# lturing/tacotronv2_wavernn_chinese

Measured on AMD Instinct MI355X. Metric: audio ksamples/sec (22.05 kHz, 10-bit RAW WaveRNN, batch=1 per GPU), higher is better.
Workload: dtype f32

## Files before the change

### tacotronv2_wavernn_chinese_amd/csrc/loop_team2.hip

```cpp
#include "device_util.h"
#include "wrnn_internal.h"

#define T2_WGS 32
#define T2_THREADS 512
#define T2_SPIN_MAX 300000u

typedef unsigned long long u64;

namespace {

__device__ __forceinline__ unsigned xcc_id2() {
    unsigned v;
    asm volatile("s_getreg_b32 %0, hwreg(HW_REG_XCC_ID)" : "=s"(v));
    return v & 0xf;
}

__device__ __forceinline__ void st_granule(u64 *base, unsigned idx, unsigned tag, unsigned payload) {
    const u64 v = ((u64)tag << 32) | payload;
    const unsigned off = idx * 8u;
    asm volatile("global_store_dwordx2 %0, %1, %2" ::"v"(off), "v"(v), "s"(base) : "memory");
}
template <int N>
__device__ __forceinline__ void peek_n(const u64 *base, unsigned idx, unsigned stride, u64 (&g)[N]) {
#pragma unroll
    for (int i = 0; i < N; ++i) g[i] = __hip_atomic_load(base + idx + (unsigned)i * stride, __ATOMIC_RELAXED, __HIP_MEMORY_SCOPE_AGENT);
}
template <int N, int SHIFT>
__device__ __forceinline__ bool tags_ok(const u64 (&g)[N], unsigned tag) {
    bool ok = true;
#pragma unroll
    for (int i = 0; i < N; ++i) ok = ok && ((unsigned)(g[i] >> SHIFT) == tag);
    return ok;
}
template <int N, int SHIFT>
__device__ __forceinline__ void finish_n(const u64 *base, unsigned idx, unsigned stride, unsigned tag, u64 (&g)[N], bool &dead,
                                         unsigned *err, unsigned code) {
    unsigned spins = 0;
    while (!dead && !__all(tags_ok<N, SHIFT>(g, tag))) {
        if (++spins > T2_SPIN_MAX) { dead = true; if ((threadIdx.x & 63) == 0) atomicExch(err, code); break; }
        peek_n<N>(base, idx, stride, g);
    }
}

#ifndef T2_STAGGER
#define T2_STAGGER 3
#endif
#ifndef T2_DEFER_OUT
#define T2_DEFER_OUT 0
#endif
#ifndef T2_PRESLEEP
#define T2_PRESLEEP 0
#endif
#ifndef T2_LATE_B
#define T2_LATE_B 2
#endif
__device__ __forceinline__ unsigned take_granule(const u64 *base, unsigned idx, unsigned tag, bool &dead, unsigned *err, unsigned code, u64 (&gb)[1]) {
    u64 ga[1];
#if T2_PRESLEEP
    __builtin_amdgcn_s_sleep(T2_PRESLEEP);
#endif
    peek_n<1>(base, idx, 1, ga);
#if T2_LATE_B == 2
    finish_n<1, 32>(base, idx, 1, tag, ga, dead, err, code);
    return (unsigned)ga[0];
#else
    __builtin_amdgcn_s_sleep(T2_STAGGER);
    peek_n<1>(base, idx, 1, gb);
    if (__all(tags_ok<1, 32>(ga, tag))) {
        unsigned r = (unsigned)ga[0];
#if T2_LATE_B
        asm volatile("" : "+v"(r));
#endif
        return r;
    }
#if T2_LATE_B
    if (__all(tags_ok<1, 32>(gb, tag))) { unsigned r = (unsigned)gb[0]; asm volatile("" : "+v"(r)); return r; }
    u64 gc[1];
    peek_n<1>(base, idx, 1, gc);
    finish_n<1, 32>(base, idx, 1, tag, gc, dead, err, code);
    unsigned r = (unsigned)gc[0];
    asm volatile("" : "+v"(r));
    return r;
#else
    finish_n<1, 32>(base, idx, 1, tag, gb, dead, err, code);
    return (unsigned)gb[0];
#endif
#endif
}
__device__ __forceinline__ void retire_look(u64 (&gb)[1]) {
#if T2_LATE_B
    asm volatile("" ::"v"(gb[0]));
#endif
}

template <int CTRL>
__device__ __forceinline__ float dpp_get(float v) {
    return __int_as_float(__builtin_amdgcn_update_dpp(0, __float_as_int(v), CTRL, 0xf, 0xf, true));
}
__device__ __forceinline__ float row_sum(float v) {
    v += dpp_get<0xB1>(v);
    v += dpp_get<0x4E>(v);
    v += dpp_get<0x141>(v);
    v += dpp_get<0x140>(v);
    return v;
}
__device__ __forceinline__ float wave_max(float v) {
    asm volatile(
        "s_nop 1\n\t"
        "v_max_f32_dpp %0, %0, %0 quad_perm:[1,0,3,2] row_mask:0xf bank_mask:0xf\n\t"
        "s_nop 1\n\t"
        "v_max_f32_dpp %0, %0, %0 quad_perm:[2,3,0,1] row_mask:0xf bank_mask:0xf\n\t"
        "s_nop 1\n\t"
        "v_max_f32_dpp %0, %0, %0 row_half_mirror row_mask:0xf bank_mask:0xf\n\t"
        "s_nop 1\n\t"
        "v_max_f32_dpp %0, %0, %0 row_mirror row_mask:0xf bank_mask:0xf\n\t"
        "s_nop 1\n\t"
        "v_max_f32_dpp %0, %0, %0 row_bcast:15 row_mask:0xa bank_mask:0xf\n\t"
        "s_nop 1\n\t"
        "v_max_f32_dpp %0, %0, %0 row_bcast:31 row_mask:0xc bank_mask:0xf\n\t"
        "s_nop 1"
        : "+v"(v));
    return v;
}

#define XB_PLANE 68
#define XB_VEC (8 * XB_PLANE)
__device__ __forceinline__ int perm(int j) { return ((j >> 2) & 7) * XB_PLANE + (j >> 5) * 4 + (j & 3); }

typedef float f2 __attribute__((ext_vector_type(2)));
__device__ __forceinline__ f2 mk2(float a, float b) { f2 r; r.x = a; r.y = b; return r; }
__device__ __forceinline__ f2 pkfma(f2 a, f2 b, f2 c) { return __builtin_elementwise_fma(a, b, c); }

__device__ __forceinline__ void dot32x3(const float *w, const float *vec, int q, float &o0, float &o1, float &o2) {
    const float4 *p = (const float4 *)vec + q;
    f2 a = mk2(0.f, 0.f), b = mk2(0.f, 0.f), c = mk2(0.f, 0.f);
#pragma unroll
    for (int h = 0; h < 2; ++h) {
        float4 x[4];
#pragma unroll
        for (int k = 0; k < 4; ++k) x[k] = p[(4 * h + k) * (XB_PLANE / 4)];
#pragma unroll
        for (int k = 0; k < 4; ++k) {
            const int kk = 4 * h + k;
            const f2 xl = mk2(x[k].x, x[k].y), xh = mk2(x[k].z, x[k].w);
            a = pkfma(mk2(w[4 * kk + 0], w[4 * kk + 1]), xl, a);
            b = pkfma(mk2(w[32 + 4 * kk + 0], w[32 + 4 * kk + 1]), xl, b);
            c = pkfma(mk2(w[64 + 4 * kk + 0], w[64 + 4 * kk + 1]), xl, c);
            a = pkfma(mk2(w[4 * kk + 2], w[4 * kk + 3]), xh, a);
            b = pkfma(mk2(w[32 + 4 * kk + 2], w[32 + 4 * kk + 3]), xh, b);
            c = pkfma(mk2(w[64 + 4 * kk + 2], w[64 + 4 * kk + 3]), xh, c);
        }
    }
    o0 = a.x + a.y; o1 = b.x + b.y; o2 = c.x + c.y;
}
__device__ __forceinline__ void dot32x3_mixed(const float *w, const float4 *wl_, const float *vec, int q, float &o0, float &o1, float &o2) {
    const float4 *p = (const float4 *)vec + q;
    f2 a = mk2(0.f, 0.f), b = mk2(0.f, 0.f), c = mk2(0.f, 0.f);
#pragma unroll
    for (int h = 0; h < 2; ++h) {
        float4 x[4], wn[4];
#pragma unroll
        for (int k = 0; k < 4; ++k) { x[k] = p[(4 * h + k) * (XB_PLANE / 4)]; wn[k] = wl_[(4 * h + k) * 256]; }
#pragma unroll
        for (int k = 0; k < 4; ++k) {
            const int kk = 4 * h + k;
            const f2 xl = mk2(x[k].x, x[k].y), xh = mk2(x[k].z, x[k].w);
            a = pkfma(mk2(w[4 * kk + 0], w[4 * kk + 1]), xl, a);
            b = pkfma(mk2(w[32 + 4 * kk + 0], w[32 + 4 * kk + 1]), xl, b);
            c = pkfma(mk2(wn[k].x, wn[k].y), xl, c);
            a = pkfma(mk2(w[4 * kk + 2], w[4 * kk + 3]), xh, a);
            b = pkfma(mk2(w[32 + 4 * kk + 2], w[32 + 4 * kk + 3]), xh, b);
            c = pkfma(mk2(wn[k].z, wn[k].w), xh, c);
        }
    }
    o0 = a.x + a.y; o1 = b.x + b.y; o2 = c.x + c.y;
}
__device__ __forceinline__ float dot32(const float *w, const float *vec, int q) {
    const float4 *p = (const float4 *)vec + q;
    f2 s0 = mk2(0.f, 0.f), s1 = mk2(0.f, 0.f);
    float4 x[8];
#pragma unroll
    for (int k = 0; k < 8; ++k) x[k] = p[k * (XB_PLANE / 4)];
#pragma unroll
    for (int k = 0; k < 8; ++k) {
        s0 = pkfma(mk2(w[4 * k + 0], w[4 * k + 1]), mk2(x[k].x, x[k].y), s0);
        s1 = pkfma(mk2(w[4 * k + 2], w[4 * k + 3]), mk2(x[k].z, x[k].w), s1);
    }
    return (s0.x + s0.y) + (s1.x + s1.y);
}
__device__ __forceinline__ float sigmoid_fast(float x) { return __builtin_amdgcn_rcpf(1.0f + __expf(-x)); }
__device__ __forceinline__ float tanh_fast(float x) { return 1.0f - 2.0f * __builtin_amdgcn_rcpf(__expf(2.0f * x) + 1.0f); }

constexpr int L_COND = 0;
constexpr int L_CSTA = L_COND + 512 * 4;
constexpr int L_GH1 = L_CSTA + 512 * 4;
constexpr int L_CSTQ = L_GH1 + 1536;
constexpr int L_HAND = L_CSTQ + 256;
constexpr int L_MISC = L_HAND + 128;
constexpr int L_XB = L_MISC + 64;
constexpr int XB_H1 = 0, XB_X2 = 1, XB_X3 = 2, XB_H2 = 3, XB_F1 = 4, XB_F2 = 5;
constexpr int L_SW = L_XB + 6 * XB_VEC;
constexpr int L_FC3 = L_SW + 8 * 256 * 4;
constexpr int L_TOTAL = L_FC3 + 16384;
static_assert(L_TOTAL * 4 <= 163840, "LDS budget");
constexpr int M_XF = 9, M_DEAD = 10;

constexpr unsigned G_X3 = 0, G_F1 = 1024, G_F2 = 2048, G_PR = 3072, G_GH = 4096;

}

#define P2(i)                                                               \
    do {                                                                    \
        if (PROF) {                                                         \
            const u64 now_ = __builtin_readcyclecounter();                  \
            prof_acc[i] += now_ - prof_last;                                \
            prof_last = now_;                                               \
        }                                                                   \
    } while (0)

template <int MODE, bool PROF, bool RAGGED>
__global__ void __launch_bounds__(T2_THREADS, 2) loop_team2_kernel(WrnnTeamArgs a) {
    extern __shared__ __attribute__((aligned(16))) char smem[];
    float *lds = (float *)smem;
    float *xb = lds + L_XB;
    float *gh1s = lds + L_GH1;
    int *misc_i = (int *)(lds + L_MISC);
    float *misc_f = lds + L_MISC;

    const int tid = threadIdx.x;
    const int lane = tid & 63, wave = __builtin_amdgcn_readfirstlane(tid >> 6);
    const bool isC = wave < 4;
    const int wl = wave & 3;
    if (isC) __builtin_amdgcn_s_setprio(3);
    const int r4 = lane >> 4, q = lane & 15;
    const WrnnDims d = a.d;
    const int NC = d.NC, HOP = d.HOP, T = a.T;
    const float4 *swl = (const float4 *)(lds + L_SW) + (tid - 256);

    if (tid == 0) {
        const unsigned x = xcc_id2();
        misc_i[M_DEAD] = 0;
        const unsigned rank = atomicAdd(&a.ctl[x], 1u);
        unsigned slot1 = 0, arrived = 0;
        if (rank == 0) {
            slot1 = atomicAdd(&a.ctl[8], 1u) + 1u;
            __hip_atomic_store(&a.ctl[16 + x], slot1, __ATOMIC_RELAXED, __HIP_MEMORY_SCOPE_AGENT);
        }
        for (unsigned spins = 0; spins < WRNN_ARRIVE_POLLS; ++spins) {
            slot1 = __hip_atomic_load(&a.ctl[16 + x], __ATOMIC_RELAXED, __HIP_MEMORY_SCOPE_AGENT);
            arrived = __hip_atomic_load(&a.ctl[x], __ATOMIC_RELAXED, __HIP_MEMORY_SCOPE_AGENT);
            if (slot1 && arrived >= T2_WGS) break;
        }
        if (arrived < T2_WGS) { slot1 = 0; if (rank < T2_WGS) atomicCAS(a.err, 0u, WRNN_DEVERR_BUSY); }
        misc_i[0] = slot1 ? (int)slot1 - 1 : 1 << 20;
        misc_i[1] = (int)rank;
    }
    __syncthreads();
    const int team = __builtin_amdgcn_readfirstlane(misc_i[0]);
    const int g = __builtin_amdgcn_readfirstlane(misc_i[1]);
    __syncthreads();
    if (g >= T2_WGS || team >= a.n_teams || team >= a.n_rows) return;
    u64 *mail = a.mail + (size_t)team * WRNN_TEAM_MAIL_GRANULES;

    const int unit = 16 * g + 4 * wl + r4;
    const int qslot = wl * 4 + r4;
    const int c3row0 = 32 * g + 8 * wl + 2 * r4;
    const bool has_fc3 = c3row0 < NC;

    float wv[160];
    {
        const float *src = a.team_w + (size_t)g * WRNN_TEAM_NWREG * WRNN_TEAM_THREADS + (wl * 64 + lane);
        if (isC) {
#pragma unroll
            for (int i = 0; i < 96; ++i) wv[i] = src[(size_t)(96 + i) * WRNN_TEAM_THREADS];
#pragma unroll
            for (int i = 0; i < 64; ++i) wv[96 + i] = src[(size_t)(288 + i) * WRNN_TEAM_THREADS];
        } else {
#pragma unroll
            for (int i = 0; i < 96; ++i) wv[i] = src[(size_t)i * WRNN_TEAM_THREADS];
#pragma unroll
            for (int i = 0; i < 64; ++i) wv[96 + i] = src[(size_t)(192 + i) * WRNN_TEAM_THREADS];
#pragma unroll
            for (int k = 0; k < 8; ++k)
                ((float4 *)(lds + L_SW))[k * 256 + (tid - 256)] =
                    make_float4(src[(size_t)(256 + 4 * k) * WRNN_TEAM_THREADS], src[(size_t)(257 + 4 * k) * WRNN_TEAM_THREADS],
                                src[(size_t)(258 + 4 * k) * WRNN_TEAM_THREADS], src[(size_t)(259 + 4 * k) * WRNN_TEAM_THREADS]);
        }
        const float4 *f3 = (const float4 *)(a.team_fc3 + (size_t)g * 16384);
        float4 *dst = (float4 *)(lds + L_FC3);
        for (int i = tid; i < 4096; i += T2_THREADS) dst[i] = f3[i];
        ((float4 *)(lds + L_CSTA))[tid] = make_float4(a.wI0[tid], a.u1[tid], a.u1[512 + tid], a.u1[1024 + tid]);
        if (!isC && q == 0) {
            float *cq = lds + L_CSTQ + qslot * 16;
            cq[0] = a.w[a.off.r1_bhh + unit]; cq[1] = a.w[a.off.r1_bhh + 512 + unit]; cq[2] = a.w[a.off.r1_bhh + 1024 + unit];
            cq[3] = a.w[a.off.r2_bhh + unit]; cq[4] = a.w[a.off.r2_bhh + 512 + unit]; cq[5] = a.w[a.off.r2_bhh + 1024 + unit];
            cq[6] = has_fc3 ? a.w[a.off.fc3_b + c3row0] : 0.0f;
            cq[7] = (c3row0 + 1 < NC) ? a.w[a.off.fc3_b + c3row0 + 1] : 0.0f;
        }
    }
    __syncthreads();
    float *cstQ = lds + L_CSTQ + qslot * 16;
    float *hand = lds + L_HAND + qslot * 8;
    const int pj = perm(tid), pu = perm(unit);
    const int sidx = tid - 256;

    bool dead = false;
    unsigned epoch = 0;
    u64 prof_acc[17] = {0};
    u64 prof_last = 0;

    for (int it = team; it < (RAGGED ? a.n_slots : a.n_rows); it += a.n_teams) {
        int row = it;
        if constexpr (RAGGED) {
            row = a.sched[it];
            if (row < 0) continue;
        }
        const WrnnRow rw = a.rows[row];
        int64_t seg_end = a.seg0 + a.seg_len;
        if constexpr (RAGGED) {
            if (a.seg0 >= rw.steps) continue;
            if (seg_end > rw.steps) seg_end = rw.steps;
        }
        const bool resume = a.seg0 > 0;
        float *st = a.state + (size_t)row * WRNN_TEAM_STATE_FLOATS;
        const float4 *CONDg = (const float4 *)a.tabCOND + ((size_t)row * a.seg_len - (size_t)a.seg0) * 512;
        const float *C2g = a.tabC2 + (size_t)rw.utt * (T + 1) * 1536;
        const float *C3g = a.tabC3 + (size_t)rw.utt * (T + 1) * 512;
        const float *C4g = a.tabC4 + (size_t)rw.utt * (T + 1) * 512;

        float h1_j = resume ? st[tid] : 0.0f;
        float xfeed = resume ? st[4096] : (a.x_init ? a.x_init[row] : 0.0f);
        xb[XB_H2 * XB_VEC + pj] = resume ? st[512 + tid] : 0.0f;
        for (int i = tid; i < 1536; i += T2_THREADS) gh1s[i] = resume ? st[1024 + i] : a.w[a.off.r1_bhh + i];
        if (tid == 0) misc_f[M_XF] = xfeed;
        const int64_t pos0 = rw.start + a.seg0;
        int nfi = (int)(pos0 / HOP), nph = (int)(pos0 - (int64_t)nfi * HOP);
        int cst_frame = -1000000;
        int pend_frame = -1;
        float nzE0 = 0.f, nzE1 = 0.f, nzn0 = 0.f, nzn1 = 0.f;
        float4 cnext0 = make_float4(0.f, 0.f, 0.f, 0.f), cnext1 = cnext0;

        auto s_prepare = [&](int64_t ts, unsigned ep_of_ts) {
            const bool live = nfi < T;
            const int fi = live ? nfi : T;
            if (++nph == HOP) { nph = 0; ++nfi; }
            pend_frame = fi;
            ((float4 *)(lds + L_COND))[sidx] = cnext0;
            ((float4 *)(lds + L_COND))[sidx + 256] = cnext1;
        };
        auto s_prefetch = [&](int64_t ts) {
            if (ts < seg_end) {
                cnext0 = CONDg[(size_t)ts * 512 + sidx];
                cnext1 = CONDg[(size_t)ts * 512 + sidx + 256];
            }
        };
        auto s_noise = [&](int64_t ts, unsigned ep_of_ts) {
            if (MODE == WRNN_MODE_MOL && wave == 4 && lane <= NC / 3) {
                const int nr = NC / 3;
                float u;
                if (a.noise_mode == WRNN_NOISE_INJECTED)
                    u = lane < nr ? a.noise1[((size_t)ts * a.n_rows + row) * nr + lane] : a.noise2[(size_t)ts * a.n_rows + row];
                else
                    u = 1e-5f + wrnn_uniform(a.seed, (uint64_t)ts, (uint32_t)row, (uint32_t)lane) * (1.0f - 2e-5f);
                misc_f[32 + 16 * (ep_of_ts & 1u) + lane] = lane < nr ? -logf(-logf(u)) : logf(u) - logf(1.0f - u);
            }
            if (MODE == WRNN_MODE_RAW && has_fc3) {
                float nz0 = 0.f, nz1 = 0.f;
                if (a.noise_mode == WRNN_NOISE_INJECTED) {
                    const float *qp = a.noise1 + ((size_t)ts * a.n_rows + row) * NC + c3row0;
                    nz0 = -logf(qp[0]); nz1 = -logf(qp[1]);
                    if (q == 0) { hand[4 + 2 * (ep_of_ts & 1u)] = nz0; hand[5 + 2 * (ep_of_ts & 1u)] = nz1; }
                } else if (a.noise_mode == WRNN_NOISE_PHILOX) {
                    if ((ts & 31) == 0) {
                        const Philox4 pz = wrnn_raw_block(a.seed, (uint64_t)ts + 2u * (unsigned)q, (uint32_t)row, (uint32_t)c3row0);
                        nzE0 = -__logf(-logf(u01_from_bits(pz.x)));
                        nzE1 = -__logf(-logf(u01_from_bits(pz.y)));
                        nzn0 = -__logf(-logf(u01_from_bits(pz.z)));
                        nzn1 = -__logf(-logf(u01_from_bits(pz.w)));
                    }
                    if (q == (int)((ts >> 1) & 15)) {
                        const bool odd = (ts & 1) != 0;
                        hand[4 + 2 * (ep_of_ts & 1u)] = odd ? nzn0 : nzE0;
                        hand[5 + 2 * (ep_of_ts & 1u)] = odd ? nzn1 : nzE1;
                    }
                } else if (q == 0) { hand[4 + 2 * (ep_of_ts & 1u)] = 0.f; hand[5 + 2 * (ep_of_ts & 1u)] = 0.f; }
            }
        };
        auto s_frame_consts = [&]() {
            if (pend_frame >= 0 && pend_frame != cst_frame) {
                if (q == 0) {
                    const int fi = pend_frame;
                    cstQ[8] = C2g[(size_t)fi * 1536 + unit]; cstQ[9] = C2g[(size_t)fi * 1536 + 512 + unit];
                    cstQ[10] = C2g[(size_t)fi * 1536 + 1024 + unit];
                    cstQ[11] = C3g[(size_t)fi * 512 + unit];
                    cstQ[12] = C4g[(size_t)fi * 512 + unit];
                }
                cst_frame = pend_frame;
            }
        };
        if (!isC) {
            if (q == 0) {
                hand[0] = resume ? st[2560 + unit] : cstQ[3];
                hand[1] = resume ? st[2560 + 512 + unit] : cstQ[4];
                hand[2] = resume ? st[2560 + 1024 + unit] : cstQ[5];
            }
            s_prefetch(a.seg0);
            s_prepare(a.seg0, epoch + 1);
            s_prefetch(a.seg0 + 1);
            s_noise(a.seg0, epoch + 1);
            s_frame_consts();
        }
        __syncthreads();

        int out_k = 0;
        float out_x = 0.0f;
        u64 lookb[1] = {0};
        for (int64_t t = a.seg0; t < seg_end; ++t) {
            ++epoch;
            const unsigned par = epoch & 1u;
            if (PROF) prof_last = __builtin_readcyclecounter();

            float x2_j;
            {
                const float4 cA = ((const float4 *)(lds + L_CSTA))[tid];
                const float4 cd = ((const float4 *)(lds + L_COND))[tid];
                const float ghr = gh1s[tid], ghz = gh1s[512 + tid], ghn = gh1s[1024 + tid];
                const float xprev = xfeed;
                const float xin = fmaf(cA.x, xprev, cd.x);
                const float rg = sigmoid_fast(fmaf(cA.y, xprev, cd.y) + ghr);
                const float zg = sigmoid_fast(fmaf(cA.z, xprev, cd.z) + ghz);
                const float ng = tanh_fast(fmaf(cA.w, xprev, cd.w) + rg * ghn);
                h1_j = (1.0f - zg) * ng + zg * h1_j;
                x2_j = xin + h1_j;
                xb[XB_H1 * XB_VEC + pj] = h1_j;
                xb[XB_X2 * XB_VEC + pj] = x2_j;
            }
            P2(0);
            __syncthreads();
            P2(1);

            if (isC) {
                const float h2o = xb[XB_H2 * XB_VEC + pu];
                const float x2u = xb[XB_X2 * XB_VEC + pu];
                const float g2r = hand[0], g2z = hand[1], g2n = hand[2];
                const float c2r = cstQ[8], c2z = cstQ[9], c2n = cstQ[10];
                float gr, gz, gn;
                dot32x3(wv, xb + XB_X2 * XB_VEC, q, gr, gz, gn);
                gr = row_sum(gr) + c2r; gz = row_sum(gz) + c2z; gn = row_sum(gn) + c2n;
                const float rg = sigmoid_fast(gr + g2r);
                const float zg = sigmoid_fast(gz + g2z);
                const float ng = tanh_fast(gn + rg * g2n);
                const float x3u = x2u + ((1.0f - zg) * ng + zg * h2o);
                if (q == 0) st_granule(mail, G_X3 + par * 512 + unit, epoch, __float_as_uint(x3u));
            } else {
                if (T2_DEFER_OUT && MODE == WRNN_MODE_RAW && g == 0 && tid == 256 && t > a.seg0) {
                    if (a.labels_out) a.labels_out[(size_t)row * a.steps + t - 1] = out_k;
                    a.samples_out[(size_t)row * a.steps + t - 1] = out_x;
                }
                float sr, sz, sn;
                __builtin_amdgcn_s_sleep(2);
                dot32x3(wv, xb + XB_H1 * XB_VEC, q, sr, sz, sn);
                sr = row_sum(sr) + cstQ[0]; sz = row_sum(sz) + cstQ[1]; sn = row_sum(sn) + cstQ[2];
                if (q == 0) {
                    st_granule(mail, G_GH + par * 1536 + unit, epoch, __float_as_uint(sr));
                    st_granule(mail, G_GH + par * 1536 + 512 + unit, epoch, __float_as_uint(sz));
                    st_granule(mail, G_GH + par * 1536 + 1024 + unit, epoch, __float_as_uint(sn));
                }
            }
            P2(2);
            {
                const float x3 = __uint_as_float(take_granule(mail, G_X3 + par * 512 + tid, epoch, dead, a.err, 11u, lookb));
                xb[XB_X3 * XB_VEC + pj] = x3;
                xb[XB_H2 * XB_VEC + pj] = x3 - x2_j;
            }
            P2(3);
            __syncthreads();
            retire_look(lookb);
            P2(4);

            if (isC) {
                const float s = row_sum(dot32(wv + 128, xb + XB_X3 * XB_VEC, q)) + cstQ[11];
                if (q == 0) st_granule(mail, G_F1 + par * 512 + unit, epoch, __float_as_uint(fmaxf(s, 0.0f)));
            } else {
                if (t + 1 < seg_end) s_noise(t + 1, epoch + 1);
            }
            P2(5);
            {
                xb[XB_F1 * XB_VEC + pj] = __uint_as_float(take_granule(mail, G_F1 + par * 512 + tid, epoch, dead, a.err, 12u, lookb));
            }
            P2(6);
            __syncthreads();
            retire_look(lookb);
            P2(7);

            if (isC) {
                const float s = row_sum(dot32(wv + 96, xb + XB_F1 * XB_VEC, q)) + cstQ[12];
                if (q == 0) st_granule(mail, G_F2 + par * 512 + unit, epoch, __float_as_uint(fmaxf(s, 0.0f)));
            } else {
                if (t + 1 < seg_end) s_prepare(t + 1, epoch + 1);
            }
            P2(8);
            {
                xb[XB_F2 * XB_VEC + pj] = __uint_as_float(take_granule(mail, G_F2 + par * 512 + tid, epoch, dead, a.err, 13u, lookb));
            }
            P2(9);
            __syncthreads();
            retire_look(lookb);
            P2(10);

            if (isC) {
                float lg0, lg1;
                {
                    const float4 *xp = (const float4 *)(xb + XB_F2 * XB_VEC) + q;
                    const float4 *wp = (const float4 *)(lds + L_FC3) + (size_t)(wl * 2) * 8 * 64 + lane;
                    f2 pa = mk2(0.f, 0.f), pb = mk2(0.f, 0.f);
#pragma unroll
                    for (int kk = 0; kk < 8; kk += 4) {
                        float4 x[4], wa[4], wb[4];
#pragma unroll
                        for (int k = 0; k < 4; ++k) { x[k] = xp[(kk + k) * (XB_PLANE / 4)]; wa[k] = wp[(kk + k) * 64]; wb[k] = wp[(8 + kk + k) * 64]; }
#pragma unroll
                        for (int k = 0; k < 4; ++k) {
                            const f2 xl = mk2(x[k].x, x[k].y), xh = mk2(x[k].z, x[k].w);
                            pa = pkfma(mk2(wa[k].x, wa[k].y), xl, pa); pb = pkfma(mk2(wb[k].x, wb[k].y), xl, pb);
                            pa = pkfma(mk2(wa[k].z, wa[k].w), xh, pa); pb = pkfma(mk2(wb[k].z, wb[k].w), xh, pb);
                        }
                    }
                    lg0 = row_sum(pa.x + pa.y) + cstQ[6];
                    lg1 = row_sum(pb.x + pb.y) + cstQ[7];
                }
                if (a.logits_out && q == 0 && has_fc3) {
                    float *lo = a.logits_out + ((size_t)t * a.n_rows + row) * NC + c3row0;
                    lo[0] = lg0;
                    if (c3row0 + 1 < NC) lo[1] = lg1;
                }
                if (MODE == WRNN_MODE_RAW) {
                    const float v0 = has_fc3 ? lg0 + hand[4 + 2 * par] : -INFINITY;
                    const float v1 = (c3row0 + 1 < NC) ? lg1 + hand[5 + 2 * par] : -INFINITY;
                    const bool p1 = v1 > v0;
                    if (q == 0) st_granule(mail, G_PR + par * 512 + 16 * g + qslot,
                                           (epoch << 10) | (unsigned)(p1 ? c3row0 + 1 : c3row0), __float_as_uint(p1 ? v1 : v0));
                    P2(13);
                    {
                        __builtin_amdgcn_s_sleep(3);
                        u64 gq[2];
                        peek_n<2>(mail, G_PR + par * 512 + wl * 128 + lane * 2, 1, gq);
                        finish_n<2, 42>(mail, G_PR + par * 512 + wl * 128 + lane * 2, 1, epoch & 0x3fffffu, gq, dead, a.err, 14u);
                        P2(14);
                        const float va = __uint_as_float((unsigned)gq[0]), vb = __uint_as_float((unsigned)gq[1]);
                        const bool pb_ = vb > va;
                        const float best = pb_ ? vb : va;
                        const int besti = (int)(((pb_ ? gq[1] : gq[0]) >> 32) & 1023u);
                        const float mx = __int_as_float(__builtin_amdgcn_readlane(__float_as_int(wave_max(best)), 63));
                        const u64 ball = __ballot(best == mx);
                        const int src = (int)__builtin_ctzll(ball ? ball : 1ull);
                        const int k = __builtin_amdgcn_readlane(besti, src);
                        if (lane == 0) { misc_f[16 + 2 * wl] = mx; misc_i[17 + 2 * wl] = k; }
                    }
                } else {
                    if (q == 0 && has_fc3) {
                        st_granule(mail, G_PR + par * 512 + c3row0, epoch, __float_as_uint(lg0));
                        if (c3row0 + 1 < NC) st_granule(mail, G_PR + par * 512 + c3row0 + 1, epoch, __float_as_uint(lg1));
                    }
                    if (wave == 0) {
                        const int nr = NC / 3;
                        float mylg = 0.0f;
                        if (lane < NC) {
                            u64 gq[1];
                            peek_n<1>(mail, G_PR + par * 512 + lane, 1, gq);
                            unsigned spins = 0;
                            while (!dead && (unsigned)(gq[0] >> 32) != epoch) {
                                if (++spins > T2_SPIN_MAX) { dead = true; atomicExch(a.err, 16u); break; }
                                peek_n<1>(mail, G_PR + par * 512 + lane, 1, gq);
                            }
                            mylg = __uint_as_float((unsigned)gq[0]);
                        }
                        const float v = lane < nr ? mylg + misc_f[32 + 16 * par + lane] : -INFINITY;
                        const float mx = __int_as_float(__builtin_amdgcn_readlane(__float_as_int(wave_max(v)), 63));
                        const u64 ball = __ballot(v == mx);
                        const int km = (int)__builtin_ctzll(ball ? ball : 1ull);
                        const float mean = __int_as_float(__builtin_amdgcn_readlane(__float_as_int(mylg), nr + km));
                        const float ls = fmaxf(__int_as_float(__builtin_amdgcn_readlane(__float_as_int(mylg), 2 * nr + km)), -32.23619130191664f);
                        float xs = mean + expf(ls) * misc_f[32 + 16 * par + nr];
                        xs = fminf(fmaxf(xs, -1.0f), 1.0f);
                        if (lane == 0) {
                            float xf = xs;
                            if (a.x_forced) { float v = a.x_forced[(size_t)t * a.n_rows + row]; asm volatile("" : "+v"(v)); xf = v; }
                            misc_f[M_XF] = xf;
                            if (g == 0) {
                                if (a.labels_out) a.labels_out[(size_t)row * a.steps + t] = km;
                                a.samples_out[(size_t)row * a.steps + t] = xs;
                            }
                        }
                    }
                }
            } else {
                s_frame_consts();
                s_prefetch(t + 2);
                u64 gq[6];
                peek_n<6>(mail, G_GH + par * 1536 + sidx, 256, gq);
                finish_n<6, 32>(mail, G_GH + par * 1536 + sidx, 256, epoch, gq, dead, a.err, 15u);
#pragma unroll
                for (int m = 0; m < 6; ++m) gh1s[sidx + m * 256] = __uint_as_float((unsigned)gq[m]);
                P2(13);
                {
                    float sr, sz, sn;
                    dot32x3_mixed(wv + 96, swl, xb + XB_H2 * XB_VEC, q, sr, sz, sn);
                    sr = row_sum(sr) + cstQ[3]; sz = row_sum(sz) + cstQ[4]; sn = row_sum(sn) + cstQ[5];
                    if (q == 0) { hand[0] = sr; hand[1] = sz; hand[2] = sn; }
                }
            }
            P2(11);
            __syncthreads();
            P2(12);
            if (MODE == WRNN_MODE_RAW) {
                const float4 m0 = *(const float4 *)(misc_f + 16), m1 = *(const float4 *)(misc_f + 20);
                float bv = m0.x; int bk = __float_as_int(m0.y);
                if (m0.z > bv) { bv = m0.z; bk = __float_as_int(m0.w); }
                if (m1.x > bv) { bv = m1.x; bk = __float_as_int(m1.y); }
                if (m1.z > bv) { bv = m1.z; bk = __float_as_int(m1.w); }
                const float x_new = 2.0f * (float)bk / ((float)NC - 1.0f) - 1.0f;
                xfeed = x_new;
                if (a.x_forced) { float v = a.x_forced[(size_t)t * a.n_rows + row]; asm volatile("" : "+v"(v)); xfeed = v; }
                out_k = bk; out_x = x_new;
#if !T2_DEFER_OUT
                if (g == 0 && tid == 0) {
                    if (a.labels_out) a.labels_out[(size_t)row * a.steps + t] = bk;
                    a.samples_out[(size_t)row * a.steps + t] = x_new;
                }
#endif
            } else {
                xfeed = misc_f[M_XF];
            }
            if ((t & 63) == 63) {
                if (dead && lane == 0) misc_i[M_DEAD] = 1;
                __syncthreads();
                if (misc_i[M_DEAD]) return;
            }
        }
        __syncthreads();
        if (T2_DEFER_OUT && MODE == WRNN_MODE_RAW && g == 0 && tid == 256 && seg_end > a.seg0) {
            if (a.labels_out) a.labels_out[(size_t)row * a.steps + seg_end - 1] = out_k;
            a.samples_out[(size_t)row * a.steps + seg_end - 1] = out_x;
        }
        if (seg_end < (RAGGED ? (int64_t)a.rows[row].steps : a.steps)) {
            if (g == 0) {
                st[tid] = h1_j;
                st[512 + tid] = xb[XB_H2 * XB_VEC + pj];
                for (int i = tid; i < 1536; i += T2_THREADS) st[1024 + i] = gh1s[i];
                if (tid == 0) st[4096] = xfeed;
            }
            if (!isC && q == 0) { st[2560 + unit] = hand[0]; st[2560 + 512 + unit] = hand[1]; st[2560 + 1024 + unit] = hand[2]; }
        }
    }
    if (PROF && a.prof && lane == 0 && g == 0 && team == 0) {
        for (int i = 0; i < 17; ++i) a.prof[wave * WRNN_PROF_SLOTS + i] += prof_acc[i];
    }
}

static const void *team2_fn(int mode, bool prof, bool ragged) {
    if (mode == WRNN_MODE_RAW) {
        if (ragged) return (const void *)loop_team2_kernel<WRNN_MODE_RAW, false, true>;
        return prof ? (const void *)loop_team2_kernel<WRNN_MODE_RAW, true, false> : (const void *)loop_team2_kernel<WRNN_MODE_RAW, false, false>;
    }
    return ragged ? (const void *)loop_team2_kernel<WRNN_MODE_MOL, false, true> : (const void *)loop_team2_kernel<WRNN_MODE_MOL, false, false>;
}

hipError_t wrnn_team2_occupancy(int mode, bool prof, int *blocks_per_cu, size_t *lds_bytes) {
    const size_t lds = (size_t)L_TOTAL * sizeof(float);
    *lds_bytes = lds;
    int worst = 1 << 30;
    for (int ragged = 0; ragged < 2; ++ragged) {
        const void *fn = team2_fn(mode, prof, ragged != 0);
        hipError_t e = hipFuncSetAttribute(fn, hipFuncAttributeMaxDynamicSharedMemorySize, (int)lds);
        if (e != hipSuccess) return e;
        int blocks = 0;
        e = hipOccupancyMaxActiveBlocksPerMultiprocessor(&blocks, fn, T2_THREADS, lds);
        if (e != hipSuccess) return e;
        if (blocks < worst) worst = blocks;
    }
    *blocks_per_cu = worst;
    return hipSuccess;
}

hipError_t wrnn_launch_loop_team2(const WrnnTeamArgs &a, hipStream_t s) {
    (void)hipGetLastError();
    const size_t lds = (size_t)L_TOTAL * sizeof(float);
    const bool ragged = a.ragged != 0, prof = a.prof != nullptr && a.d.mode == WRNN_MODE_RAW && !ragged;
    const void *fn = team2_fn(a.d.mode, prof, ragged);
    hipError_t e = hipFuncSetAttribute(fn, hipFuncAttributeMaxDynamicSharedMemorySize, (int)lds);
    if (e != hipSuccess) return e;
    void *args[] = {(void *)&a};
    return hipLaunchKernel(fn, dim3(a.n_teams * 32), dim3(T2_THREADS), args, lds, s);
}
```

Before: 301.9.

## Pre-reduce argmax per wave and poll candidates from a single wave

Each wave now reduces its quad candidates to one per-wave max before publishing, so only 128 granules are written per parity instead of 512. Only wave 0 polls the mailbox, using one dwordx4 load per lane with an all-lanes ready check, and writes the single global winner to LDS. The sample value comes from a precomputed LDS lookup table instead of being computed after the barrier. This shortens the cross-workgroup argmax exchange and the post-barrier merge, but the other waves no longer help with polling and the tie-breaking order may change.

```diff
diff --git a/tacotronv2_wavernn_chinese_amd/csrc/loop_team2.hip b/tacotronv2_wavernn_chinese_amd/csrc/loop_team2.hip
--- a/tacotronv2_wavernn_chinese_amd/csrc/loop_team2.hip
+++ b/tacotronv2_wavernn_chinese_amd/csrc/loop_team2.hip
@@ -123,6 +123,30 @@
     return v;
 }
 
+__device__ __forceinline__ float rows_max(float v) {
+    asm volatile(
+        "s_nop 1\n\t"
+        "v_max_f32_dpp %0, %0, %0 row_bcast:15 row_mask:0xa bank_mask:0xf\n\t"
+        "s_nop 1\n\t"
+        "v_max_f32_dpp %0, %0, %0 row_bcast:31 row_mask:0xc bank_mask:0xf\n\t"
+        "s_nop 1"
+        : "+v"(v));
+    return v;
+}
+
+typedef unsigned u4 __attribute__((ext_vector_type(4)));
+#ifndef T2_RACE_SLEEP
+#define T2_RACE_SLEEP 3
+#endif
+__device__ __forceinline__ u4 race_load(const u64 *base, unsigned off) {
+    u4 g;
+    asm volatile("global_load_dwordx4 %0, %1, %2 sc1\n\t"
+                 "s_waitcnt vmcnt(0)"
+                 : "=&v"(g) : "v"(off), "s"(base) : "memory");
+    return g;
+}
+__device__ __forceinline__ bool race_ok(const u4 &g, unsigned tag) { return (g.y >> 10) == tag && (g.w >> 10) == tag; }
+
 #define XB_PLANE 68
 #define XB_VEC (8 * XB_PLANE)
 __device__ __forceinline__ int perm(int j) { return ((j >> 2) & 7) * XB_PLANE + (j >> 5) * 4 + (j & 3); }
@@ -201,7 +225,8 @@
 constexpr int XB_H1 = 0, XB_X2 = 1, XB_X3 = 2, XB_H2 = 3, XB_F1 = 4, XB_F2 = 5;
 constexpr int L_SW = L_XB + 6 * XB_VEC;
 constexpr int L_FC3 = L_SW + 8 * 256 * 4;
-constexpr int L_TOTAL = L_FC3 + 16384;
+constexpr int L_XTAB = L_FC3 + 16384;
+constexpr int L_TOTAL = L_XTAB + 1024;
 static_assert(L_TOTAL * 4 <= 163840, "LDS budget");
 constexpr int M_XF = 9, M_DEAD = 10;
 
@@ -289,6 +314,8 @@
         const float4 *f3 = (const float4 *)(a.team_fc3 + (size_t)g * 16384);
         float4 *dst = (float4 *)(lds + L_FC3);
         for (int i = tid; i < 4096; i += T2_THREADS) dst[i] = f3[i];
+        if (MODE == WRNN_MODE_RAW)
+            for (int k = tid; k < 1024; k += T2_THREADS) lds[L_XTAB + k] = 2.0f * (float)k / ((float)NC - 1.0f) - 1.0f;
         ((float4 *)(lds + L_CSTA))[tid] = make_float4(a.wI0[tid], a.u1[tid], a.u1[512 + tid], a.u1[1024 + tid]);
         if (!isC && q == 0) {
             float *cq = lds + L_CSTQ + qslot * 16;
@@ -538,24 +565,35 @@
                     const float v0 = has_fc3 ? lg0 + hand[4 + 2 * par] : -INFINITY;
                     const float v1 = (c3row0 + 1 < NC) ? lg1 + hand[5 + 2 * par] : -INFINITY;
                     const bool p1 = v1 > v0;
-                    if (q == 0) st_granule(mail, G_PR + par * 512 + 16 * g + qslot,
-                                           (epoch << 10) | (unsigned)(p1 ? c3row0 + 1 : c3row0), __float_as_uint(p1 ? v1 : v0));
+                    const float bq = p1 ? v1 : v0;
+                    const int kq = p1 ? c3row0 + 1 : c3row0;
+                    const float mw = __int_as_float(__builtin_amdgcn_readlane(__float_as_int(rows_max(bq)), 63));
+                    const u64 bw = __ballot(bq == mw);
+                    const int kw = __builtin_amdgcn_readlane(kq, (int)__builtin_ctzll(bw ? bw : 1ull));
+                    if (lane == 0) st_granule(mail, G_PR + par * 512 + 4 * g + wl, (epoch << 10) | (unsigned)kw, __float_as_uint(mw));
                     P2(13);
-                    {
-                        __builtin_amdgcn_s_sleep(3);
-                        u64 gq[2];
-                        peek_n<2>(mail, G_PR + par * 512 + wl * 128 + lane * 2, 1, gq);
-                        finish_n<2, 42>(mail, G_PR + par * 512 + wl * 128 + lane * 2, 1, epoch & 0x3fffffu, gq, dead, a.err, 14u);
+                    if (wave == 0) {
+                        if (T2_RACE_SLEEP) __builtin_amdgcn_s_sleep(T2_RACE_SLEEP);
+                        const unsigned roff = (G_PR + par * 512 + 2u * (unsigned)lane) * 8u;
+                        const unsigned rtag = epoch & 0x3fffffu;
+                        u4 gq = race_load(mail, roff);
+                        for (unsigned spins = 0; !dead && !__all(race_ok(gq, rtag));) {
+                            if (++spins > T2_SPIN_MAX) { dead = true; if (lane == 0) atomicExch(a.err, 14u); break; }
+                            gq = race_load(mail, roff);
+                        }
                         P2(14);
-                        const float va = __uint_as_float((unsigned)gq[0]), vb = __uint_as_float((unsigned)gq[1]);
+                        const float va = __uint_as_float(gq.x), vb = __uint_as_float(gq.z);
                         const bool pb_ = vb > va;
                         const float best = pb_ ? vb : va;
-                        const int besti = (int)(((pb_ ? gq[1] : gq[0]) >> 32) & 1023u);
+                        const int besti = (int)((pb_ ? gq.w : gq.y) & 1023u);
+                        const float bestx = lds[L_XTAB + besti];
                         const float mx = __int_as_float(__builtin_amdgcn_readlane(__float_as_int(wave_max(best)), 63));
                         const u64 ball = __ballot(best == mx);
                         const int src = (int)__builtin_ctzll(ball ? ball : 1ull);
-                        const int k = __builtin_amdgcn_readlane(besti, src);
-                        if (lane == 0) { misc_f[16 + 2 * wl] = mx; misc_i[17 + 2 * wl] = k; }
+                        if (lane == 0) {
+                            misc_i[16] = __builtin_amdgcn_readlane(__float_as_int(bestx), src);
+                            misc_i[17] = __builtin_amdgcn_readlane(besti, src);
+                        }
                     }
                 } else {
                     if (q == 0 && has_fc3) {
@@ -614,12 +652,10 @@
             __syncthreads();
             P2(12);
             if (MODE == WRNN_MODE_RAW) {
-                const float4 m0 = *(const float4 *)(misc_f + 16), m1 = *(const float4 *)(misc_f + 20);
-                float bv = m0.x; int bk = __float_as_int(m0.y);
-                if (m0.z > bv) { bv = m0.z; bk = __float_as_int(m0.w); }
-                if (m1.x > bv) { bv = m1.x; bk = __float_as_int(m1.y); }
-                if (m1.z > bv) { bv = m1.z; bk = __float_as_int(m1.w); }
-                const float x_new = 2.0f * (float)bk / ((float)NC - 1.0f) - 1.0f;
+                const float2 win = *(const float2 *)(misc_f + 16);
+                const float x_new = win.x;
+                const int bk = __float_as_int(win.y);
+                P2(15);
                 xfeed = x_new;
                 if (a.x_forced) { float v = a.x_forced[(size_t)t * a.n_rows + row]; asm volatile("" : "+v"(v)); xfeed = v; }
                 out_k = bk; out_x = x_new;
```

New measurement: 305.5, median of 6. 1.2% higher.
